# remmel/OcclusionFusion

Measured on AMD Instinct MI355X. Metric: fusion frames/sec (warp+integrate+solve), 640x480 depth -> 512^3 TSDF, higher is better.
Workload: dtype f32/f64

## Files before the change

occlusionfusion_amd/csrc/gn.hip:

```cpp
#include <math.h>
#include <stdlib.h>
#include <string.h>
#include <algorithm>
#include <chrono>
#include <array>
#include <condition_variable>
#include <memory>
#include <mutex>
#include <thread>
#include <type_traits>
#include <utility>
#include <cstdlib>
#include <cstdio>
#include <vector>

#include "ofx_common.h"

namespace ofx {

constexpr int kBlk = 256;
#ifndef OFX_KPROJ
#define OFX_KPROJ 4
#endif
constexpr int kProj = OFX_KPROJ;
// ... 1699 lines not shown
        const double z = M[a][b] / (dr[a] * dc[b]);
        const double err = (double)(float)h16(z) - z;
        e2 += 2.0 * err * err;
      }
    }
  s_e[t] = e2;
  __syncthreads();
  if (t < 64) {
    double sum = 0.0;
    for (int i = t; i < T; i += 64) sum += s_e[i];
    sum = wave_sum(sum);
    if (t == 0) s_sig = sqrt(sum) + 0x1p-10;
  }
  __syncthreads();
  OFX_AS_STAMP(3)
  const double sig = s_sig;
  auto b16 = [](_Float16 h) { return __builtin_bit_cast(uint16_t, h); };
#pragma unroll
  for (int a = 0; a < NA; ++a)
#pragma unroll
    for (int b = 0; b < NB; ++b) {
      const int R = tr + TR * a, C = tc + TC * b;
      if (R >= n || C >= kAsD) continue;
      if (C >= n) {
        s_z[R * kAsD + C] = 0;
      } else if (R == C) {
        s_z[R * kAsD + C] = b16(bad ? (_Float16)(R < 6 * kCS ? 1.0f : 0.0f) : h16(1.0 + sig));
      } else if (R < C) {
        const uint16_t h = b16(bad ? (_Float16)0.0f : h16(M[a][b] / (dr[a] * dc[b])));
        s_z[R * kAsD + C] = h;
        s_z[C * kAsD + R] = h;
      }
    }
  if (tc == 0)
#pragma unroll
    for (int a = 0; a < NA; ++a) {
      const int R = tr + TR * a;
      if (R < kAsD) g.as_dsc[(int64_t)c * kAsD + R] = R < n ? (float)dr[a] : 0.f;
      if (R < kAsD && g.as_one) as_tab_at(g.as_tab, g.as_tab_cap).dsc[(int64_t)c * kAsD + R] = R < n ? (float)dr[a] : 0.f;
      if (R < n) g.as_rsc[s_dst[R]] = (float)dr[a];
    }
  __syncthreads();
  OFX_AS_STAMP(4)
  for (int i = t; i < n * kAsK; i += T) {
    const int R = i / kAsK, k = i % kAsK;
    const int d = s_dst[R], cp = d / kAsRS, rs = d % kAsRS;
    reinterpret_cast<uint4*>(g.as_slab)[((int64_t)cp * kAsK + k) * kAsRS + rs] =
        reinterpret_cast<const uint4*>(s_z + R * kAsD)[k];
  }
  if (g.as_one) {
    uint4* sl = as_tab_at(g.as_tab, g.as_tab_cap).slab + (int64_t)c * kAsK * kAsD;
    for (int i = t; i < n * kAsK; i += T) {
      const int k = i / n, R = i - k * n;
      sl[(int64_t)k * kAsD + R] = reinterpret_cast<const uint4*>(s_z + R * kAsD)[k];
    }
  }
  if (t < kCS) g.racc[c * kCS + t] = 0.0;
  OFX_AS_STAMP(5)
#undef OFX_AS_STAMP
}

typedef double as_d4 __attribute__((ext_vector_type(4)));
constexpr int kNT = (kAsD + 15) / 16, kNP = 16 * kNT, kInvT = 64 * kNT;
__device__ __forceinline__ void as_invert_mfma(const GnDev& g, const double* __restrict__ A, int c, int t) {
  constexpr int kPanel = 16 * kNP;
  constexpr int kGJ = (2 * kPanel + 2 * 16 * 17) * 8, kZ = kAsD * kAsD * 2;
  __shared__ __attribute__((aligned(16))) char s_buf[kGJ > kZ ? kGJ : kZ];
  __shared__ int s_dom[kAsDN];
  __shared__ int s_sl[kAsDN][kAsDN];
  __shared__ int s_dst[kAsD];
  __shared__ double s_d[kNP], s_e[kInvT];
  __shared__ double s_sig;
  double* s_C = reinterpret_cast<double*>(s_buf);
  double* s_P = s_C + 2 * kPanel;
  uint16_t* s_z = reinterpret_cast<uint16_t*>(s_buf);
  const int l = t & 63, lr = l >> 4, lc = l & 15;
  const int w = __builtin_amdgcn_readfirstlane(t >> 6);
#ifdef OFX_STAMPS
#define OFX_AS_STAMP(k) \
  if (t == 0 && g.stamps) g.stamps[((int64_t)63 * g.nwg_row + c) * 8 + (k)] = __builtin_amdgcn_s_memtime();
#else
#define OFX_AS_STAMP(k)
#endif
  OFX_AS_STAMP(0)
  if (t < kAsDN) s_dom[t] = g.as_dom[c * kAsDN + t];
  if (t < kAsD) s_dst[t] = g.as_dst[(int64_t)c * kAsD + t];
  __syncthreads();
  int nd = 0;
  for (int i = 0; i < kAsDN; ++i) nd += s_dom[i] >= 0 ? 1 : 0;
  for (int q = t; q < kAsDN * kAsDN; q += kInvT) {
    const int i = q / kAsDN, j = q % kAsDN;
    s_sl[i][j] = (i < nd && j < nd) ? g.map[(int64_t)s_dom[i] * g.N + s_dom[j]] - 1 : -1;
  }
  __syncthreads();
  const int n = 6 * nd;
  const int C0 = 16 * w + lc;
  auto slot = [&](int R, int C) { return (R < n && C < n) ? s_sl[min(R / 6, kAsDN - 1)][min(C / 6, kAsDN - 1)] : -1; };
  as_d4 acc[kNT];
#pragma unroll
  for (int i = 0; i < kNT; ++i)
#pragma unroll
    for (int r = 0; r < 4; ++r) {
      const int R = 16 * i + lr + 4 * r;
      const int sl = slot(R, C0);
      acc[i][r] = A[36 * (int64_t)(sl >= 0 ? sl : 0) + 6 * (R % 6) + C0 % 6];
      if (r == 3) __builtin_amdgcn_sched_barrier(0);
    }
// ... 105 lines not shown
  __syncthreads();
  auto h16 = [](double z) -> _Float16 { return (_Float16)(float)z; };
  auto b16 = [](_Float16 h) { return __builtin_bit_cast(uint16_t, h); };
  double e2 = 0.0;
  const double dC = s_d[C0];
#pragma unroll
  for (int i = 0; i < kNT; ++i)
#pragma unroll
    for (int r = 0; r < 4; ++r) {
      const int R = 16 * i + lr + 4 * r;
      if (R >= n || C0 >= kAsD) continue;
      if (C0 >= n) {
        s_z[R * kAsD + C0] = 0;
      } else if (R < C0) {
        const double z = bad ? 0.0 : acc[i][r] / (s_d[R] * dC);
        const _Float16 h = h16(z);
        const double err = (double)(float)h - z;
        e2 += 2.0 * err * err;
        s_z[R * kAsD + C0] = b16(h);
        s_z[C0 * kAsD + R] = b16(h);
      }
      if (r == 3) __builtin_amdgcn_sched_barrier(0);
    }
  s_e[t] = e2;
  __syncthreads();
  if (t < 64) {
    double sum = 0.0;
    for (int i = t; i < kInvT; i += 64) sum += s_e[i];
    sum = wave_sum(sum);
    if (t == 0) s_sig = sqrt(sum) + 0x1p-10;
  }
  __syncthreads();
  OFX_AS_STAMP(3)
  const double sig = s_sig;
  if (t < n) s_z[t * kAsD + t] = b16(bad ? (_Float16)(t < 6 * kCS ? 1.0f : 0.0f) : h16(1.0 + sig));
  if (t < kAsD) {
    const double dr = s_d[t];
    g.as_dsc[(int64_t)c * kAsD + t] = t < n ? (float)dr : 0.f;
    if (g.as_one) as_tab_at(g.as_tab, g.as_tab_cap).dsc[(int64_t)c * kAsD + t] = t < n ? (float)dr : 0.f;
    if (t < n) g.as_rsc[s_dst[t]] = (float)dr;
  }
  __syncthreads();
  OFX_AS_STAMP(4)
  for (int i = t; i < n * kAsK; i += kInvT) {
    const int R = i / kAsK, k = i % kAsK;
    const int d = s_dst[R], cp = d / kAsRS, rs = d % kAsRS;
    reinterpret_cast<uint4*>(g.as_slab)[((int64_t)cp * kAsK + k) * kAsRS + rs] =
        reinterpret_cast<const uint4*>(s_z + R * kAsD)[k];
  }
  if (g.as_one) {
    uint4* sl = as_tab_at(g.as_tab, g.as_tab_cap).slab + (int64_t)c * kAsK * kAsD;
    for (int i = t; i < n * kAsK; i += kInvT) {
      const int k = i / n, R = i - k * n;
      sl[(int64_t)k * kAsD + R] = reinterpret_cast<const uint4*>(s_z + R * kAsD)[k];
    }
  }
  if (t < kCS) g.racc[c * kCS + t] = 0.0;
  OFX_AS_STAMP(5)
#undef OFX_AS_STAMP
}

constexpr int kAsInvTC = 16;
template <bool kMfma>
__global__ __launch_bounds__(kMfma ? kInvT : 16 * kAsInvTC) void k_as_invert(GnDev g, const double* __restrict__ A,
                                                                                   const double* __restrict__ rhs) {
  const int c = blockIdx.x, t = threadIdx.x;
  if (g.flags[F_STOPPED]) return;
  if constexpr (kMfma) as_invert_mfma(g, A, c, t);
  else as_invert_body<16, kAsInvTC>(g, A, c, t);
  if (!g.warm_now && t < 6 * kCS) {
    const int64_t o = 6 * (int64_t)c * kCS + t;
    const double v[V_N] = {0.0, rhs[o], 0.0, 0.0, 0.0, 0.0, 0.0, 0.0};
    store_rec(g.st, o, v);
  }
  if (c == 0 && t == 0) { g.flags[F_DONE] = 0; g.flags[F_PCG_IT] = 0; g.flags[F_PCG_CNT] = 0; g.flags[F_REFRESH] = 0; }
}

template <bool kTest, int kL>
__global__ __launch_bounds__(kAsRS * kL) void k_as_apply(const int32_t* stopw, const int32_t* meta, const int32_t* gat,
                                                        const uint16_t* slab, const double* in, double* out,
                                                        const int32_t* src, const float* dsc, const float* rsc) {
  constexpr int kT = kAsRS * kL;
  constexpr int kG = (kAsGat + kT - 1) / kT;
  constexpr int kKL = (kAsK + kL - 1) / kL;
  __shared__ __attribute__((aligned(16))) double s_w[kAsSrc * kAsD];
  __shared__ double s_seg[kAsRS];
  const int c = blockIdx.x, t = threadIdx.x, lane = t & 63;
  const int sg = t / kL, hl = t % kL;
  const int32_t* mt = meta + (int64_t)c * kAsMeta;
  int stop = 0;
  if (kTest) stop = stopw[(int64_t)c * 64 + lane];
  const int nrs = mt[0];
  int gn[kG], sv[kG];
#pragma unroll
  for (int j = 0; j < kG; ++j) {
    const int i = min(kT * j + t, kAsGat - 1);
    gn[j] = gat[(int64_t)c * kAsGat + i];
    sv[j] = src[c * kAsSrc + min(i / kAsDN, kAsSrc - 1)];
  }
  const int sl = mt[64 + sg];
  const float rscale = rsc[(int64_t)c * kAsRS + sg];
  const int rr = t < 6 * kCS ? t : 6 * kCS - 1;
  const int o0 = mt[2 + rr], o1 = mt[3 + rr];
  asm volatile("" ::: "memory");
  if (kTest) {
    stop = __builtin_amdgcn_readfirstlane(stop);
    if (stop != 0) return;
// ... 836 lines not shown
  double thr_new = 0.0, th_cur = 1e300;
  auto shift = [](int s) {
    const int e = s < 40 ? s : 2 * s - 40;
    const int k = e & 3;
    const double c = k == 0 ? 1.0 : k == 1 ? 0.84089641525371454303 : k == 2 ? 0.70710678118654752440
                                                                            : 0.59460355750136053336;
    return ldexp(c, -(e >> 2));
  };
  if (wv == 0 && hw == 0 && etol > 0.0) {
    const double rca = 1.0 / alpha;
    const double diag = kFirst ? rca : rca + beta * ralpha_prev;
    const double e2 = kFirst ? 0.0 : beta * ralpha_prev * ralpha_prev;
    const double sig = shift(lane);
    double d = (diag - sig) - (kFirst ? 0.0 : e2 / sd.x);
    if (fabs(d) < 1e-300) d = -1e-300;
    const double c = (kFirst ? 0.0 : sd.y) + (d < 0.0 ? 1.0 : 0.0);
    sd_new = make_double2(d, c);
    const uint64_t free_ = __ballot(c == 0.0);
    const double th = free_ ? shift(__ffsll((unsigned long long)free_) - 1) : 0.0;
    th_cur = th;
    const double tu = fmin(th, th_prev);
    thr_new = (etol * etol) * tu;
  }
  auto lead_stores = [&]() {
    if (lead) {
      sc_w[kScAlpha + 2 + par_] = 1.0 / alpha; sc_w[kScGamma + 2 + par_] = 1.0 / gam; flags_w[F_PCG_CNT] = cnt + 1;
      sc_w[kScAlpha + 4 + par_] = thr_new;
      if (etol > 0.0) sc_w[kScScal + S_TH_CUR] = th_cur;
    }
    if (wv == 0 && hw == 0 && etol > 0.0) reinterpret_cast<double2*>(sc_w + kScSturm)[lane] = sd_new;
    if (kFirst && lead) sc_w[kScScal + S_BB] = bb;
  };
  OFX_STAMP(2)
  OFX_STAMPX(6)
  double nc;
  if (kWave) {
#pragma unroll
    for (int j = 0; j < kNB; ++j) {
      const bool ok = (j ? bl1 : bl0).x >= 0;
      const int slot = kW2 ? 64 * hw + lane : j * 64 + lane;
      double x[6];
#pragma unroll
      for (int k = 0; k < 3; ++k) { x[2 * k] = xb[j][k].x; x[2 * k + 1] = xb[j][k].y; }
#pragma unroll
      for (int i = 0; i < 6; ++i) {
        const double2 b01 = ab[j][3 * i], b23 = ab[j][3 * i + 1], b45 = ab[j][3 * i + 2];
        const double t = fma(b45.y, x[5], fma(b45.x, x[4], fma(b23.y, x[3], fma(b23.x, x[2], fma(b01.y, x[1], b01.x * x[0])))));
        s_prod[slot * 6 + i] = ok ? t : 0.0;
      }
    }
    OFX_STAMP(3)
    if (kW2) {
      __builtin_amdgcn_s_waitcnt(0xC07F);
      __builtin_amdgcn_s_barrier();
    } else {
      wave_lds_sync();
    }
    const int len = b1 - b0;
    const double* sp = s_prod + (b0 - wb0) * 6 + qc;
    double tv[kRowMax];
#pragma unroll
    for (int k = 0; k < kRowMax; ++k) tv[k] = sp[6 * k];
    __builtin_amdgcn_sched_barrier(0);
    double a = 0.0;
#pragma unroll
    for (int k = 0; k < kRowMax; ++k) a += k < len ? tv[k] : 0.0;
    nc = a;
  } else {
    double n[6];
    row_spmv(g, b0, b1, q, mc, n);
    nc = pick6(n, qc);
  }
  OFX_STAMP(4)
  double d[kPcgStreams] = {0.0, 0.0, 0.0, 0.0};
  {
    const double zz = fma(beta, v[V_Z], nc);
    const double qq = fma(beta, v[V_Q], m);
    const double sv = fma(beta, v[V_S], v[V_W]);
    const double p = fma(beta, v[V_P], v[V_U]);
    const double rn = fma(-alpha, sv, v[V_R]);
    const double un = fma(-alpha, qq, v[V_U]);
    const double w2 = fma(-alpha, zz, v[V_W]);
    if (own) {
      const double nv[V_N] = {fma(alpha, p, v[V_X]), rn, un, zz, qq, sv, p, w2};
      if (w0) store_rec(stw, o, nv);
      if (kAS) {
        if (w0) reinterpret_cast<__attribute__((address_space(1))) double*>(addr(mcl_v))[o] = w2;
      } else {
        s_v[hw][6 * r + q] = w2;
      }
      d[0] = rn * un; d[1] = w2 * un; d[2] = rn * rn; d[3] = p * p;
    }
  }
  OFX_STAMP(5)
  if (!kAS) wave_lds_sync();
  if constexpr (kAS) {
  } else if (kW2) {
    double hsum = 0.0;
    if (own) {
      double2 vv[kCD / 4];
      const double2* sv2 = reinterpret_cast<const double2*>(&s_v[hw][4 * (kCD / 8) * hw]);
#pragma unroll
      for (int i = 0; i < kCD / 4; ++i) vv[i] = sv2[i];
      __builtin_amdgcn_sched_barrier(0);
      double a[4] = {0.0, 0.0, 0.0, 0.0};
#pragma unroll
      for (int kk = 0; kk < kCD / 8; ++kk) {
        const float4 t = mreg[kk];
        a[0] = fma((double)t.x, vv[2 * kk].x, a[0]);
        a[1] = fma((double)t.y, vv[2 * kk].y, a[1]);
        a[2] = fma((double)t.z, vv[2 * kk + 1].x, a[2]);
        a[3] = fma((double)t.w, vv[2 * kk + 1].y, a[3]);
      }
      hsum = (a[0] + a[1]) + (a[2] + a[3]);
    }
    if (hw == 1) s_half[lane] = hsum;
    __builtin_amdgcn_s_waitcnt(0xC07F);
    __builtin_amdgcn_s_barrier();
    if (w0 && own) mn[o] = hsum + s_half[lane];
  } else if (own) {
    double a[4] = {0.0, 0.0, 0.0, 0.0};
#pragma unroll
    for (int k = 0; k < kCD / 4; ++k) {
      const float4 t = mreg[k];
      a[0] = fma((double)t.x, s_v[0][4 * k], a[0]);
      a[1] = fma((double)t.y, s_v[0][4 * k + 1], a[1]);
      a[2] = fma((double)t.z, s_v[0][4 * k + 2], a[2]);
      a[3] = fma((double)t.w, s_v[0][4 * k + 3], a[3]);
    }
    mn[o] = (a[0] + a[1]) + (a[2] + a[3]);
  }
  OFX_STAMP(6)
  if (!w0) {
    if (kW2) {
      const double s2 = wave_sum(d[2]), s3 = wave_sum(d[3]);
      if (lane == 0) { Pn[2 * ns + wv] = s2; Pn[3 * ns + wv] = s3; }
    }
    return;
  }
  d[0] = wave_sum(d[0]);
  d[1] = wave_sum(d[1]);
  if (!kW2) { d[2] = wave_sum(d[2]); d[3] = wave_sum(d[3]); }
  if (lane == 0) {
    Pn[wv] = d[0]; Pn[ns + wv] = d[1];
    if (!kW2) { Pn[2 * ns + wv] = d[2]; Pn[3 * ns + wv] = d[3]; }
  }
  lead_stores();
  OFX_STAMP(7)
}

__device__ __forceinline__ void as_lds_barrier() {
  __builtin_amdgcn_s_waitcnt(0xC07F);
  __builtin_amdgcn_s_barrier();
}
#ifdef OFX_STAMPS
#define OFX_AS_ITER_STAMP(k, cn) \
  if (lane == 0 && g.stamps && (cn) < 64) g.stamps[((int64_t)(cn) * nwg + c) * 8 + (k)] = __builtin_amdgcn_s_memtime();
#else
#define OFX_AS_ITER_STAMP(k, cn)
#endif
template <bool kFirst, int kU, bool kRowSplit>
__global__ __launch_bounds__(kAsIterT) void k_as_iter(const int32_t* stopw, const double* Pc, const double* st,
                                                      const double* sc, const char* tab, int cap, int xcd_per, int nwg,
                                                      int ep, const PcgIt* gp, int gn_iter) {
  const PcgIt& g = *gp;
  constexpr int kNs = 128 * kU;
  constexpr int kS2W = 5 * 64;
  __shared__ __attribute__((aligned(16))) double s_m[kGS * 6];
  __shared__ __attribute__((aligned(16))) double s_prod[(kGB + kRowMax) * 6];
  __shared__ __attribute__((aligned(16))) double s_w[kAsD];
  __shared__ int s_leave;
  __shared__ double s_ab[2];
  const int t = threadIdx.x, lane = t & 63;
  const int wave = __builtin_amdgcn_readfirstlane(t >> 6);
  const int c = xcd_per > 0 ? (int)(blockIdx.x & 7) * xcd_per + (int)(blockIdx.x >> 3) : (int)blockIdx.x;
  if (c >= nwg) return;
  const AsTabP tp = as_tab_at(const_cast<char*>(tab), cap);
  const int par_ = (int)((reinterpret_cast<uintptr_t>(sc) >> 3) & 1);
  const double* scb = sc - par_;
  const int32_t* rt = tp.row + (int64_t)c * kGRow;
  const double* yr = tp.y + (int64_t)par_ * cap * kAsD;
  if (wave >= 8) {
    const int tb = t - kGB;
    int stop_ep = stopw[(int64_t)c * 64 + lane];
    const int nb = rt[26];
    typedef double gd2 __attribute__((ext_vector_type(2)));
    const __attribute__((address_space(1))) gd2* A2 =
        reinterpret_cast<const __attribute__((address_space(1))) gd2*>(reinterpret_cast<const uint64_t*>(scb)[kScAop]);
    if (kRowSplit) {
      constexpr int kP = (kGB * 6 + kGB - 1) / kGB;
      int2 be[kP];
#pragma unroll
      for (int j = 0; j < kP; ++j) be[j] = tp.blk[(int64_t)c * kGB + (tb + kGB * j) / 6];
      asm volatile("" ::: "memory");
      stop_ep = __builtin_amdgcn_readfirstlane(stop_ep);
      if (stop_ep != 0) return;
      double2 ar[kP][3];
#pragma unroll
      for (int j = 0; j < kP; ++j)
        if (tb - lane + kGB * j < 6 * nb)
#pragma unroll
          for (int k = 0; k < 3; ++k) {
            const gd2 x = A2[18 * (int64_t)be[j].x + 3 * ((tb + kGB * j) % 6) + k];
            ar[j][k] = make_double2(x.x, x.y);
          }
      as_lds_barrier();
#pragma unroll
      for (int j = 0; j < kP; ++j) {
        const int pp = tb + kGB * j;
        if (pp < 6 * nb) {
          const int k = be[j].y >> 5;
          double x[6];
#pragma unroll
          for (int q = 0; q < 6; ++q) x[q] = s_m[6 * k + q];
          const double2 b01 = ar[j][0], b23 = ar[j][1], b45 = ar[j][2];
          s_prod[pp] = fma(b45.y, x[5], fma(b45.x, x[4], fma(b23.y, x[3], fma(b23.x, x[2], fma(b01.y, x[1], b01.x * x[0])))));
        }
      }
      as_lds_barrier();
      as_lds_barrier();
      return;
    }
    const int2 be = tp.blk[(int64_t)c * kGB + tb];
    asm volatile("" ::: "memory");
    stop_ep = __builtin_amdgcn_readfirstlane(stop_ep);
    if (stop_ep != 0) return;
    const __attribute__((address_space(1))) gd2* b = A2 + 18 * (int64_t)be.x;
    const bool any = tb - lane < nb;
    double2 ab[18];
    if (any)
#pragma unroll
      for (int k = 0; k < 18; ++k) { const gd2 x = b[k]; ab[k] = make_double2(x.x, x.y); }
    as_lds_barrier();
    if (any && tb < nb) {
      const int k = be.y >> 5;
      double x[6];
#pragma unroll
      for (int j = 0; j < 6; ++j) x[j] = s_m[6 * k + j];
#pragma unroll
      for (int i = 0; i < 6; ++i) {
        const double2 b01 = ab[3 * i], b23 = ab[3 * i + 1], b45 = ab[3 * i + 2];
        s_prod[tb * 6 + i] =
            fma(b45.y, x[5], fma(b45.x, x[4], fma(b23.y, x[3], fma(b23.x, x[2], fma(b01.y, x[1], b01.x * x[0])))));
      }
    }
    as_lds_barrier();
    as_lds_barrier();
    return;
  }
  if (wave >= 3) {
    const int ts = t - 192;
    int stop_ep = stopw[(int64_t)c * 64 + lane];
    const int k2 = ts < kGS ? ts : kGS - 1;
    const int4 cn = tp.con[(int64_t)c * kGS + k2];
    const int nd = rt[25], ns = rt[27];
    const int ry = min(ts >> 1, kAsD - 1), hl = ts & 1;
    asm volatile("" ::: "memory");
    stop_ep = __builtin_amdgcn_readfirstlane(stop_ep);
    if (stop_ep != 0) return;
    auto gather = [&](int4 e4, double mv[6]) {
      double2 cz[4][3];
      {
        const int e[4] = {e4.x, e4.y, e4.z, e4.w};
#pragma unroll
        for (int j = 0; j < 4; ++j) {
#ifndef OFX_AS_NOSKIP
          if (j == 0 || e[j] >= 0) {
#pragma unroll
            for (int k = 0; k < 3; ++k) cz[j][k] = reinterpret_cast<const double2*>(yr + e[j])[k];
          } else {
#pragma unroll
            for (int k = 0; k < 3; ++k) cz[j][k] = make_double2(0.0, 0.0);
          }
#else
          const double2* p = reinterpret_cast<const double2*>(yr + (e[j] >= 0 ? e[j] : e[0]));
#pragma unroll
          for (int k = 0; k < 3; ++k) cz[j][k] = p[k];
#endif
        }
      }
      asm volatile("" ::: "memory");
#pragma unroll
      for (int k = 0; k < 3; ++k) {
        const int e[4] = {e4.x, e4.y, e4.z, e4.w};
        double mx = 0.0, my = 0.0;
#pragma unroll
        for (int j = 0; j < 4; ++j) { mx += e[j] >= 0 ? cz[j][k].x : 0.0; my += e[j] >= 0 ? cz[j][k].y : 0.0; }
        mv[2 * k] = mx; mv[2 * k + 1] = my;
      }
    };
    if (ts - lane < ns) {
      double mv[6];
      gather(cn, mv);
      if (ts < ns)
#pragma unroll
        for (int j = 0; j < 6; ++j) s_m[6 * ts + j] = mv[j];
    }
    if (ns > kS2W)
      for (int kk = ts + kS2W; kk < ns; kk += kS2W) {
        double mv[6];
        gather(tp.con[(int64_t)c * kGS + kk], mv);
#pragma unroll
        for (int j = 0; j < 6; ++j) s_m[6 * kk + j] = mv[j];
      }
    as_lds_barrier();
    uint4 z[9];
#pragma unroll
    for (int k = 0; k < 9; ++k) z[k] = tp.slab[((int64_t)c * kAsK + 9 * hl + k) * kAsD + ry];
    const float dsc_r = tp.dsc[(int64_t)c * kAsD + ry];
    as_lds_barrier();
    as_lds_barrier();
    if (s_leave) return;
    const double2* w2p = reinterpret_cast<const double2*>(s_w);
    double a0 = 0.0, a1 = 0.0, a2 = 0.0, a3 = 0.0;
    auto lo = [](uint32_t u) { return (double)(float)__builtin_bit_cast(_Float16, (uint16_t)(u & 0xFFFFu)); };
    auto hi = [](uint32_t u) { return (double)(float)__builtin_bit_cast(_Float16, (uint16_t)(u >> 16)); };
#pragma unroll
    for (int k = 0; k < 9; ++k) {
      const int kw = 9 * hl + k;
      const double2 p0 = w2p[4 * kw], p1 = w2p[4 * kw + 1], p2 = w2p[4 * kw + 2], p3 = w2p[4 * kw + 3];
      a0 = fma(lo(z[k].x), p0.x, a0);
      a1 = fma(hi(z[k].x), p0.y, a1);
      a2 = fma(lo(z[k].y), p1.x, a2);
      a3 = fma(hi(z[k].y), p1.y, a3);
      a0 = fma(lo(z[k].z), p2.x, a0);
      a1 = fma(hi(z[k].z), p2.y, a1);
      a2 = fma(lo(z[k].w), p3.x, a2);
      a3 = fma(hi(z[k].w), p3.y, a3);
    }
    double dot = (a0 + a1) + (a2 + a3);
    dot += dpp_mov<0xB1>(dot);
    if (hl == 0 && ts < 2 * kAsD && (ts >> 1) < 6 * nd)
      tp.y[(int64_t)(par_ ^ 1) * cap * kAsD + (int64_t)c * kAsD + (ts >> 1)] = (double)dsc_r * dot;
    return;
  }
  const int jr = wave, r = lane >> 3, q = lane & 7;
#ifdef OFX_STAMPS
  const uint64_t t_entry = __builtin_amdgcn_s_memtime();
#endif
  const bool own = q < 6;
  const int qc = own ? q : 5;
  const int l = 8 * jr + r;
  const int row = c * kCS + r;
  const int64_t o = 6 * (int64_t)row + qc;
  int stop_ep = stopw[(int64_t)c * 64 + lane];
  double2 tpp[kPcgStreams][kU];
  double own_p[kPcgStreams];
  int cnt = 0;
  double2 ra = make_double2(0.0, 0.0), rtb = ra, rg = ra, sd = ra, tols = ra;
  double bb_stored = 0.0, th_prev = 0.0;
  if (jr == 0) {
#pragma unroll
    for (int k = 0; k < kPcgStreams; ++k)
#pragma unroll
      for (int u = 0; u < kU; ++u) tpp[k][u] = *reinterpret_cast<const double2*>(Pc + k * kNs + 2 * (lane + 64 * u));
#pragma unroll
    for (int k = 0; k < kPcgStreams; ++k) own_p[k] = Pc[k * kNs + c];
    cnt = reinterpret_cast<const int32_t*>(scb + kScFlags)[F_PCG_CNT];
    ra = *reinterpret_cast<const double2*>(scb + kScAlpha + 2);
    rtb = *reinterpret_cast<const double2*>(scb + kScAlpha + 4);
    rg = *reinterpret_cast<const double2*>(scb + kScGamma + 2);
    sd = reinterpret_cast<const double2*>(scb + kScSturm)[lane];
    bb_stored = scb[kScScal + S_BB];
    th_prev = scb[kScScal + S_TH_PREV];
    tols = *reinterpret_cast<const double2*>(scb + kScTol);
  }
  const int nd = rt[25];
  const int rs = rt[l], re = rt[l + 1], rk = rt[32 + l];
  const float dsc_l = tp.dsc[(int64_t)c * kAsD + 6 * l + qc];
  double v[V_N];
  double wg = 0.0, zg = 0.0;
  const int gi = (c * kAsRing + (l >= kCS ? l - kCS : 0)) * 6 + qc;
  if (jr == 0) {
    load_rec(st, o, v);
  } else if (kFirst) {
    const double* w0v = reinterpret_cast<const double*>(reinterpret_cast<const uint64_t*>(scb)[kScMcl]);
    wg = w0v[6 * (int64_t)rt[64 + l] + qc];
    zg = 0.0;
  } else {
    const double2 gz = tp.gh[gi];
    wg = gz.x;
    zg = gz.y;
  }
  asm volatile("" ::: "memory");
  stop_ep = __builtin_amdgcn_readfirstlane(stop_ep);
  if (stop_ep != 0) return;
// ... 126 lines not shown
  };
  if (c == 0 && etol > 0.0) {
    const double rca = 1.0 / alpha;
    const double diag = kFirst ? rca : rca + beta * ralpha_prev;
    const double e2 = kFirst ? 0.0 : beta * ralpha_prev * ralpha_prev;
    const double sig = shift(lane);
    double dd = (diag - sig) - (kFirst ? 0.0 : e2 / sd.x);
    if (fabs(dd) < 1e-300) dd = -1e-300;
    const double cc = (kFirst ? 0.0 : sd.y) + (dd < 0.0 ? 1.0 : 0.0);
    sd_new = make_double2(dd, cc);
    const uint64_t free_ = __ballot(cc == 0.0);
    const double th = free_ ? shift(__ffsll((unsigned long long)free_) - 1) : 0.0;
    th_cur = th;
    const double tu = fmin(th, th_prev);
    thr_new = (etol * etol) * tu;
  }
  double* Pn = const_cast<double*>(Pc) + (par_ ? -kPcgStreams : kPcgStreams) * (int64_t)kNs;
#pragma unroll
  for (int k = 0; k < kPcgStreams; ++k) d[k] = wave_sum(d[k]);
  if (lane == 0) { Pn[c] = d[0]; Pn[kNs + c] = d[1]; Pn[2 * kNs + c] = d[2]; Pn[3 * kNs + c] = d[3]; }
  double* sc_w = const_cast<double*>(scb);
  int32_t* flags_w = reinterpret_cast<int32_t*>(sc_w + kScFlags);
  if (lead) {
    sc_w[kScAlpha + 2 + par_] = 1.0 / alpha; sc_w[kScGamma + 2 + par_] = 1.0 / gam; flags_w[F_PCG_CNT] = cnt + 1;
    sc_w[kScAlpha + 4 + par_] = thr_new;
    if (etol > 0.0) sc_w[kScScal + S_TH_CUR] = th_cur;
  }
  if (c == 0 && etol > 0.0) reinterpret_cast<double2*>(sc_w + kScSturm)[lane] = sd_new;
  if (kFirst && lead) sc_w[kScScal + S_BB] = bb;
  OFX_AS_ITER_STAMP(6, cnt)
}

template <bool kGather>
__global__ __launch_bounds__(kAsIterT) void k_as_w0(GnDev g, const double* rhs, int xcd_per) {
  __shared__ __attribute__((aligned(16))) double s_m[kGS * 6];
  __shared__ __attribute__((aligned(16))) double s_prod[(kGB + kRowMax) * 6];
  __shared__ __attribute__((aligned(16))) double s_w[kAsD];
  asm volatile("" :: "s"(g.as_tab), "s"(g.as_tab_cap), "s"(g.N), "s"(g.flags), "s"(g.m1), "s"(g.Aop), "s"(g.st),
               "s"(g.stopw), "s"(g.ep), "s"(g.pcs), "s"(rhs), "s"(g.part_p), "s"(g.part_b), "s"(g.nw_pad), "s"(g.as_w));
  const int t = threadIdx.x, lane = t & 63;
  const int wave = __builtin_amdgcn_readfirstlane(t >> 6);
  const int nwg = g.N / kCS;
  const int c = xcd_per > 0 ? (int)(blockIdx.x & 7) * xcd_per + (int)(blockIdx.x >> 3) : (int)blockIdx.x;
  if (c >= nwg) return;
  const AsTabP tp = as_tab_at(g.as_tab, g.as_tab_cap);
  const int32_t* rt = tp.row + (int64_t)c * kGRow;
  const int stopped = g.flags[F_STOPPED];
  if (wave >= 8) {
    const int tb = t - kGB;
    constexpr int kP = (kGB * 6 + kGB - 1) / kGB;
    int2 be[kP];
#pragma unroll
    for (int j = 0; j < kP; ++j) be[j] = tp.blk[(int64_t)c * kGB + (tb + kGB * j) / 6];
    const int nb = rt[26];
    asm volatile("" ::: "memory");
    if (stopped) return;
    const double2* A2 = reinterpret_cast<const double2*>(g.Aop);
    double2 ar[kP][3];
#pragma unroll
    for (int j = 0; j < kP; ++j)
      if (tb - lane + kGB * j < 6 * nb)
#pragma unroll
        for (int k = 0; k < 3; ++k) ar[j][k] = A2[18 * (int64_t)be[j].x + 3 * ((tb + kGB * j) % 6) + k];
    as_lds_barrier();
#pragma unroll
    for (int j = 0; j < kP; ++j) {
      const int pp = tb + kGB * j;
      if (pp < 6 * nb) {
        const int k = be[j].y >> 5;
        double x[6];
#pragma unroll
        for (int q = 0; q < 6; ++q) x[q] = s_m[6 * k + q];
        const double2 b01 = ar[j][0], b23 = ar[j][1], b45 = ar[j][2];
        s_prod[pp] = ((b01.x * x[0] + b01.y * x[1]) + (b23.x * x[2] + b23.y * x[3])) + (b45.x * x[4] + b45.y * x[5]);
      }
    }
    as_lds_barrier();
    as_lds_barrier();
    return;
  }
  if (wave >= 3) {
    constexpr int kS2W = 5 * 64;
    const int ts = t - 192;
    const int k2 = ts < kGS ? ts : kGS - 1;
    int s2u = 0;
    int4 cn = make_int4(-1, -1, -1, -1);
    if (kGather) cn = tp.con[(int64_t)c * kGS + k2];
    else s2u = tp.s2n[(int64_t)c * kGS + k2];
    const int nd = rt[25], ns = rt[27];
    const int ry = min(ts >> 1, kAsD - 1), hl = ts & 1;
    asm volatile("" ::: "memory");
    if (stopped) return;
    const double* yr = tp.y + (int64_t)g.as_tab_cap * kAsD;
    auto gather = [&](int4 e4, int u, double mv[6]) {
      if (kGather) {
        const int e[4] = {e4.x, e4.y, e4.z, e4.w};
        double2 cz[4][3];
#pragma unroll
        for (int j = 0; j < 4; ++j) {
          if (j == 0 || e[j] >= 0) {
#pragma unroll
            for (int k = 0; k < 3; ++k) cz[j][k] = reinterpret_cast<const double2*>(yr + e[j])[k];
          } else {
#pragma unroll
            for (int k = 0; k < 3; ++k) cz[j][k] = make_double2(0.0, 0.0);
          }
        }
        asm volatile("" ::: "memory");
#pragma unroll
        for (int k = 0; k < 3; ++k) {
          double mx = 0.0, my = 0.0;
#pragma unroll
          for (int j = 0; j < 4; ++j) { mx += e[j] >= 0 ? cz[j][k].x : 0.0; my += e[j] >= 0 ? cz[j][k].y : 0.0; }
          mv[2 * k] = mx; mv[2 * k + 1] = my;
        }
      } else {
        const double2* p = reinterpret_cast<const double2*>(g.m1 + 6 * (int64_t)u);
#pragma unroll
        for (int k = 0; k < 3; ++k) { const double2 x = p[k]; mv[2 * k] = x.x; mv[2 * k + 1] = x.y; }
      }
    };
    if (ts - lane < ns) {
      double mv[6];
      gather(cn, s2u, mv);
      if (ts < ns)
#pragma unroll
        for (int k = 0; k < 6; ++k) s_m[6 * ts + k] = mv[k];
    }
    if (ns > kS2W)
      for (int kk = ts + kS2W; kk < ns; kk += kS2W) {
        double mv[6];
        gather(kGather ? tp.con[(int64_t)c * kGS + kk] : make_int4(-1, -1, -1, -1),
               kGather ? 0 : tp.s2n[(int64_t)c * kGS + kk], mv);
#pragma unroll
        for (int k = 0; k < 6; ++k) s_m[6 * kk + k] = mv[k];
      }
    as_lds_barrier();
    uint4 z[9];
#pragma unroll
    for (int k = 0; k < 9; ++k) z[k] = tp.slab[((int64_t)c * kAsK + 9 * hl + k) * kAsD + ry];
    const float dsc_r = tp.dsc[(int64_t)c * kAsD + ry];
    as_lds_barrier();
    as_lds_barrier();
    const double2* w2p = reinterpret_cast<const double2*>(s_w);
    double a0 = 0.0, a1 = 0.0, a2 = 0.0, a3 = 0.0;
    auto lo = [](uint32_t u) { return (double)(float)__builtin_bit_cast(_Float16, (uint16_t)(u & 0xFFFFu)); };
    auto hi = [](uint32_t u) { return (double)(float)__builtin_bit_cast(_Float16, (uint16_t)(u >> 16)); };
#pragma unroll
    for (int k = 0; k < 9; ++k) {
      const int kw = 9 * hl + k;
      const double2 p0 = w2p[4 * kw], p1 = w2p[4 * kw + 1], p2 = w2p[4 * kw + 2], p3 = w2p[4 * kw + 3];
      a0 = fma(lo(z[k].x), p0.x, a0);
      a1 = fma(hi(z[k].x), p0.y, a1);
      a2 = fma(lo(z[k].y), p1.x, a2);
      a3 = fma(hi(z[k].y), p1.y, a3);
      a0 = fma(lo(z[k].z), p2.x, a0);
      a1 = fma(hi(z[k].z), p2.y, a1);
      a2 = fma(lo(z[k].w), p3.x, a2);
      a3 = fma(hi(z[k].w), p3.y, a3);
    }
    double dot = (a0 + a1) + (a2 + a3);
    dot += dpp_mov<0xB1>(dot);
    if (hl == 0 && ts < 2 * kAsD && (ts >> 1) < 6 * nd)
      tp.y[(int64_t)c * kAsD + (ts >> 1)] = (double)dsc_r * dot;
    return;
  }
  const int jr = wave, r = lane >> 3, q = lane & 7;
  const bool own = q < 6;
  const int qc = own ? q : 5;
  const int l = 8 * jr + r;
  const int row = c * kCS + r;
  const int64_t o = 6 * (int64_t)row + q, oc = 6 * (int64_t)row + qc;
  const int nd = rt[25];
  const int rs = rt[l], re = rt[l + 1];
  const float dsc_l = tp.dsc[(int64_t)c * kAsD + 6 * l + qc];
  const int rk = rt[32 + l];
  double v[V_N];
  double u_as = 0.0, bo = 0.0, th_cur_old = 0.0;
  if (jr == 0) {
    load_rec(g.st, oc, v);
    if (!kGather) u_as = g.m1[oc];
    bo = rhs[oc];
    th_cur_old = g.pcs[kScScal + S_TH_CUR];
  }
  asm volatile("" ::: "memory");
  if (stopped) {
    if (jr == 0) {
      g.stopw[(int64_t)c * 64 + lane] = g.ep;
      if (c == 0 && lane == 0) w0_lead_stores(g, th_cur_old, true, true);
    }
    return;
  }
  as_lds_barrier();
  if (kGather && jr == 0) u_as = s_m[6 * rk + qc];
  as_lds_barrier();
  const int len = l < nd ? re - rs : 0;
  const double* sp = s_prod + rs * 6 + qc;
  double tv[kRowMax];
#pragma unroll
  for (int k = 0; k < kRowMax; ++k) tv[k] = sp[6 * k];
  double w = 0.0;
#pragma unroll
  for (int k = 0; k < kRowMax; ++k) w += k < len ? tv[k] : 0.0;
  double d[4] = {0.0, 0.0, 0.0, 0.0};
  if (jr == 0 && own) {
    v[V_U] = u_as;
    v[V_W] = w;
    store_rec(g.st, o, v);
    g.as_w[o] = w;
    d[0] = v[V_R] * v[V_U]; d[1] = w * v[V_U]; d[2] = v[V_R] * v[V_R]; d[3] = bo * bo;
  }
  if (own) s_w[6 * l + q] = l < nd ? w * (double)dsc_l : 0.0;
  as_lds_barrier();
  if (jr != 0) return;
#pragma unroll
  for (int k = 0; k < 4; ++k) d[k] = wave_sum(d[k]);
  const int ns = g.nw_pad;
  if (lane == 0) {
    g.part_p[c] = d[0]; g.part_p[ns + c] = d[1]; g.part_p[2 * ns + c] = d[2];
    g.part_p[3 * ns + c] = 0.0;
    g.part_b[c] = d[3];
  }
  if (c == 0)
    for (int i = nwg + lane; i < ns; i += 64) {
#pragma unroll
      for (int k = 0; k < 2 * kPcgStreams; ++k) g.part_p[k * ns + i] = 0.0;
      g.part_b[i] = 0.0;
    }
  g.stopw[(int64_t)c * 64 + lane] = 0;
  if (c == 0 && lane == 0) w0_lead_stores(g, th_cur_old, true, true);
}

template <int KU>
__global__ __launch_bounds__(512) void k_as_proj2(GnDev g, const double* rhs, int xcd_per) {
  __shared__ __attribute__((aligned(16))) double s_w[kAsD];
  __shared__ double s_c[kProj];
  __shared__ int s_fin;
  asm volatile("" :: "s"(g.as_tab), "s"(g.as_tab_cap), "s"(g.N), "s"(g.flags), "s"(g.n_prev), "s"(g.xh), "s"(g.th),
               "s"(g.part_p), "s"(g.nw_pad), "s"(g.stopw), "s"(g.ep), "s"(g.st), "s"(rhs));
  const int t = threadIdx.x, lane = t & 63;
  const int wave = __builtin_amdgcn_readfirstlane(t >> 6);
  const int nwg = g.N / kCS;
  const int c = xcd_per > 0 ? (int)(blockIdx.x & 7) * xcd_per + (int)(blockIdx.x >> 3) : (int)blockIdx.x;
  if (c >= nwg) return;
  const AsTabP tp = as_tab_at(g.as_tab, g.as_tab_cap);
  const int32_t* rt = tp.row + (int64_t)c * kGRow;
  const int stopped = g.flags[F_STOPPED];
  if (wave >= 3) {
    const int ts = t - 192;
    const int ry = min(ts >> 1, kAsD - 1), hl = ts & 1;
    const int nd = rt[25];
    uint4 z[9];
#pragma unroll
    for (int k = 0; k < 9; ++k) z[k] = tp.slab[((int64_t)c * kAsK + 9 * hl + k) * kAsD + ry];
    const float dsc_r = tp.dsc[(int64_t)c * kAsD + ry];
    asm volatile("" ::: "memory");
    if (stopped) return;
    as_lds_barrier();
    as_lds_barrier();
    const double2* w2p = reinterpret_cast<const double2*>(s_w);
    double a0 = 0.0, a1 = 0.0, a2 = 0.0, a3 = 0.0;
    auto lo = [](uint32_t u) { return (double)(float)__builtin_bit_cast(_Float16, (uint16_t)(u & 0xFFFFu)); };
    auto hi = [](uint32_t u) { return (double)(float)__builtin_bit_cast(_Float16, (uint16_t)(u >> 16)); };
#pragma unroll
    for (int k = 0; k < 9; ++k) {
      const int kw = 9 * hl + k;
      const double2 p0 = w2p[4 * kw], p1 = w2p[4 * kw + 1], p2 = w2p[4 * kw + 2], p3 = w2p[4 * kw + 3];
      a0 = fma(lo(z[k].x), p0.x, a0);
      a1 = fma(hi(z[k].x), p0.y, a1);
      a2 = fma(lo(z[k].y), p1.x, a2);
      a3 = fma(hi(z[k].y), p1.y, a3);
      a0 = fma(lo(z[k].z), p2.x, a0);
      a1 = fma(hi(z[k].z), p2.y, a1);
      a2 = fma(lo(z[k].w), p3.x, a2);
      a3 = fma(hi(z[k].w), p3.y, a3);
    }
    double dot = (a0 + a1) + (a2 + a3);
    dot += dpp_mov<0xB1>(dot);
    if (hl == 0 && ts < 2 * kAsD && (ts >> 1) < 6 * nd)
      tp.y[(int64_t)g.as_tab_cap * kAsD + (int64_t)c * kAsD + (ts >> 1)] = (double)dsc_r * dot;
    return;
  }
  const int jr = wave, r = lane >> 3, q = lane & 7;
  const bool own = q < 6;
  const int qc = own ? q : 5;
  const int l = 8 * jr + r;
  const int row = c * kCS + r;
  const int64_t o = 6 * (int64_t)row + q;
  const int nd = rt[25];
  const int64_t og = jr == 0 ? 6 * (int64_t)row + qc : 6 * (int64_t)rt[64 + l] + qc;
  const float dsc_l = tp.dsc[(int64_t)c * kAsD + 6 * l + qc];
  const int np = g.n_prev;
  const int64_t stride = 6 * (int64_t)g.N;
  const double rb = rhs[og];
  double xo[kProj], to[kProj];
#pragma unroll
  for (int j = 0; j < kProj; ++j) { xo[j] = jr == 0 ? g.xh[j * stride + og] : 0.0; to[j] = g.th[j * stride + og]; }
  double2 pt[kProjP][KU];
  if (jr == 0) load_streams2_padded<kProjP, KU>(g.part_p, g.nw_pad, pt);
  asm volatile("" ::: "memory");
  if (stopped) {
    if (jr == 0) g.stopw[(int64_t)c * 64 + lane] = g.ep;
    return;
  }
  if (jr == 0) {
    double cj[kProj];
    const bool fin = galerkin_coeffs<KU>(g, np, pt, cj);
    if (lane == 0) {
#pragma unroll
      for (int j = 0; j < kProj; ++j) s_c[j] = cj[j];
      s_fin = fin ? 1 : 0;
    }
  }
  as_lds_barrier();
  const bool fin = s_fin != 0;
  double xv = 0.0, rv = rb;
#pragma unroll
  for (int j = 0; j < kProj; ++j)
    if (j < np && fin) { const double cj = s_c[j]; xv += cj * xo[j]; rv -= cj * to[j]; }
  if (jr == 0 && own) {
    const double v[V_N] = {xv, rv, 0.0, 0.0, 0.0, 0.0, 0.0, 0.0};
    store_rec(g.st, o, v);
  }
  if (own) s_w[6 * l + q] = l < nd ? rv * (double)dsc_l : 0.0;
  as_lds_barrier();
}
// ... 1405 lines not shown
```

Before: 357.0.

## Spread the slab dot product over four lanes per row with swizzled slab layout

The per-row dot of the fp16 slab against the LDS weight vector moves from two lanes per row with uint4 loads to four lanes per row with uint2 loads. Each lane now holds 9 words and the partials are combined with two DPP reductions. The slab words are stored swizzled (y and z swapped) so each lane's uint2 pair lines up with its weights, and idle waves of the gather group take part of the dot. The intent is to lower the per-lane register load and latency of this tail, at the cost of more lanes, an extra DPP step, and a layout change every consumer of the slab must follow.

New measurement: 371.1 (median of 6 runs). 3.9% higher.

```diff
diff --git a/occlusionfusion_amd/csrc/gn.hip b/occlusionfusion_amd/csrc/gn.hip
--- a/occlusionfusion_amd/csrc/gn.hip
+++ b/occlusionfusion_amd/csrc/gn.hip
@@ -1775,7 +1775,8 @@
     uint4* sl = as_tab_at(g.as_tab, g.as_tab_cap).slab + (int64_t)c * kAsK * kAsD;
     for (int i = t; i < n * kAsK; i += T) {
       const int k = i / n, R = i - k * n;
-      sl[(int64_t)k * kAsD + R] = reinterpret_cast<const uint4*>(s_z + R * kAsD)[k];
+      const uint4 v = reinterpret_cast<const uint4*>(s_z + R * kAsD)[k];
+      sl[(int64_t)k * kAsD + R] = make_uint4(v.x, v.z, v.y, v.w);
     }
   }
   if (t < kCS) g.racc[c * kCS + t] = 0.0;
@@ -1987,7 +1988,8 @@
     uint4* sl = as_tab_at(g.as_tab, g.as_tab_cap).slab + (int64_t)c * kAsK * kAsD;
     for (int i = t; i < n * kAsK; i += kInvT) {
       const int k = i / n, R = i - k * n;
-      sl[(int64_t)k * kAsD + R] = reinterpret_cast<const uint4*>(s_z + R * kAsD)[k];
+      const uint4 v = reinterpret_cast<const uint4*>(s_z + R * kAsD)[k];
+      sl[(int64_t)k * kAsD + R] = make_uint4(v.x, v.z, v.y, v.w);
     }
   }
   if (t < kCS) g.racc[c * kCS + t] = 0.0;
@@ -2930,7 +2932,9 @@
     OFX_STAMP(3)
     if (kW2) {
       __builtin_amdgcn_s_waitcnt(0xC07F);
+      asm volatile("" ::: "memory");
       __builtin_amdgcn_s_barrier();
+      asm volatile("" ::: "memory");
     } else {
       wave_lds_sync();
     }
@@ -3029,7 +3033,64 @@
 
 __device__ __forceinline__ void as_lds_barrier() {
   __builtin_amdgcn_s_waitcnt(0xC07F);
+  asm volatile("" ::: "memory");
   __builtin_amdgcn_s_barrier();
+  asm volatile("" ::: "memory");
+}
+constexpr int kAsDotT = 4 * kAsD;
+constexpr int kDotBW = (kAsDotT - 5 * 64 + 63) / 64;
+static_assert(kDotBW >= 0 && kDotBW <= 8, "the dot's lanes fit waves 3-15");
+struct AsDotRow {
+  uint2 z[9];
+  float dsc;
+  int yd;
+};
+static_assert(kAsK == 18, "the dot's lanes take 9 words of their half each");
+__device__ __forceinline__ void as_dot_load(const AsTabP& tp, int c, int tq, AsDotRow& d) {
+  const int ry = min(tq >> 2, kAsD - 1), hl = (tq >> 1) & 1, g = tq & 1;
+  const uint2* sl = reinterpret_cast<const uint2*>(tp.slab + ((int64_t)c * kAsK + 9 * hl) * kAsD + ry) + g;
+#pragma unroll
+  for (int k = 0; k < 9; ++k) d.z[k] = sl[(int64_t)k * 2 * kAsD];
+  d.dsc = tp.dsc[(int64_t)c * kAsD + ry];
+  d.yd = c * kAsD + ry;
+}
+__device__ __forceinline__ void as_dot_cvt(const AsDotRow& d, double (&f)[36]) {
+#pragma unroll
+  for (int k = 0; k < 9; ++k) {
+    f[4 * k] = (double)(float)__builtin_bit_cast(_Float16, (uint16_t)(d.z[k].x & 0xFFFFu));
+    f[4 * k + 1] = (double)(float)__builtin_bit_cast(_Float16, (uint16_t)(d.z[k].x >> 16));
+    f[4 * k + 2] = (double)(float)__builtin_bit_cast(_Float16, (uint16_t)(d.z[k].y & 0xFFFFu));
+    f[4 * k + 3] = (double)(float)__builtin_bit_cast(_Float16, (uint16_t)(d.z[k].y >> 16));
+  }
+}
+__device__ __forceinline__ double as_dot_sum(const double (&f)[36], const double* s_w, int tq) {
+  const int hl = (tq >> 1) & 1, g = tq & 1;
+  const double2* w2p = reinterpret_cast<const double2*>(s_w) + 36 * hl + g;
+  double a = 0.0, b = 0.0;
+#pragma unroll
+  for (int k = 0; k < 9; ++k) {
+    const double2 p0 = w2p[4 * k], p2 = w2p[4 * k + 2];
+    a = fma(f[4 * k], p0.x, a);
+    b = fma(f[4 * k + 1], p0.y, b);
+    a = fma(f[4 * k + 2], p2.x, a);
+    b = fma(f[4 * k + 3], p2.y, b);
+  }
+  double dot = a + b;
+  dot += dpp_mov<0xB1>(dot);
+  dot += dpp_mov<0x4E>(dot);
+  return dot;
+}
+__device__ __forceinline__ void as_dot_tail(const AsDotRow& d, const double* s_w, const int* leave, int tq, int nd,
+                                            double* y_w) {
+  as_lds_barrier();
+  double f[36];
+  as_dot_cvt(d, f);
+#pragma unroll
+  for (int k = 0; k < 36; ++k) asm volatile("" : "+v"(f[k]));
+  as_lds_barrier();
+  if (leave && *leave) return;
+  const double dot = as_dot_sum(f, s_w, tq);
+  if ((tq & 3) == 0 && tq < kAsDotT && (tq >> 2) < 6 * nd) y_w[d.yd] = (double)d.dsc * dot;
 }
 #ifdef OFX_STAMPS
 #define OFX_AS_ITER_STAMP(k, cn) \
@@ -3061,7 +3122,7 @@
   if (wave >= 8) {
     const int tb = t - kGB;
     int stop_ep = stopw[(int64_t)c * 64 + lane];
-    const int nb = rt[26];
+    const int nb = rt[26], nd = rt[25];
     typedef double gd2 __attribute__((ext_vector_type(2)));
     const __attribute__((address_space(1))) gd2* A2 =
         reinterpret_cast<const __attribute__((address_space(1))) gd2*>(reinterpret_cast<const uint64_t*>(scb)[kScAop]);
@@ -3073,6 +3134,7 @@
       asm volatile("" ::: "memory");
       stop_ep = __builtin_amdgcn_readfirstlane(stop_ep);
       if (stop_ep != 0) return;
+      __builtin_amdgcn_s_waitcnt(0x0F70);
       double2 ar[kP][3];
 #pragma unroll
       for (int j = 0; j < kP; ++j)
@@ -3094,6 +3156,12 @@
           const double2 b01 = ar[j][0], b23 = ar[j][1], b45 = ar[j][2];
           s_prod[pp] = fma(b45.y, x[5], fma(b45.x, x[4], fma(b23.y, x[3], fma(b23.x, x[2], fma(b01.y, x[1], b01.x * x[0])))));
         }
+      }
+      if (wave < 8 + kDotBW) {
+        AsDotRow dr;
+        as_dot_load(tp, c, t - 192, dr);
+        as_dot_tail(dr, s_w, &s_leave, t - 192, nd, tp.y + (int64_t)(par_ ^ 1) * cap * kAsD);
+        return;
       }
       as_lds_barrier();
       as_lds_barrier();
@@ -3122,6 +3190,12 @@
             fma(b45.y, x[5], fma(b45.x, x[4], fma(b23.y, x[3], fma(b23.x, x[2], fma(b01.y, x[1], b01.x * x[0])))));
       }
     }
+    if (wave < 8 + kDotBW) {
+      AsDotRow dr;
+      as_dot_load(tp, c, t - 192, dr);
+      as_dot_tail(dr, s_w, &s_leave, t - 192, nd, tp.y + (int64_t)(par_ ^ 1) * cap * kAsD);
+      return;
+    }
     as_lds_barrier();
     as_lds_barrier();
     return;
@@ -3132,7 +3206,6 @@
     const int k2 = ts < kGS ? ts : kGS - 1;
     const int4 cn = tp.con[(int64_t)c * kGS + k2];
     const int nd = rt[25], ns = rt[27];
-    const int ry = min(ts >> 1, kAsD - 1), hl = ts & 1;
     asm volatile("" ::: "memory");
     stop_ep = __builtin_amdgcn_readfirstlane(stop_ep);
     if (stop_ep != 0) return;
@@ -3182,34 +3255,9 @@
         for (int j = 0; j < 6; ++j) s_m[6 * kk + j] = mv[j];
       }
     as_lds_barrier();
-    uint4 z[9];
-#pragma unroll
-    for (int k = 0; k < 9; ++k) z[k] = tp.slab[((int64_t)c * kAsK + 9 * hl + k) * kAsD + ry];
-    const float dsc_r = tp.dsc[(int64_t)c * kAsD + ry];
-    as_lds_barrier();
-    as_lds_barrier();
-    if (s_leave) return;
-    const double2* w2p = reinterpret_cast<const double2*>(s_w);
-    double a0 = 0.0, a1 = 0.0, a2 = 0.0, a3 = 0.0;
-    auto lo = [](uint32_t u) { return (double)(float)__builtin_bit_cast(_Float16, (uint16_t)(u & 0xFFFFu)); };
-    auto hi = [](uint32_t u) { return (double)(float)__builtin_bit_cast(_Float16, (uint16_t)(u >> 16)); };
-#pragma unroll
-    for (int k = 0; k < 9; ++k) {
-      const int kw = 9 * hl + k;
-      const double2 p0 = w2p[4 * kw], p1 = w2p[4 * kw + 1], p2 = w2p[4 * kw + 2], p3 = w2p[4 * kw + 3];
-      a0 = fma(lo(z[k].x), p0.x, a0);
-      a1 = fma(hi(z[k].x), p0.y, a1);
-      a2 = fma(lo(z[k].y), p1.x, a2);
-      a3 = fma(hi(z[k].y), p1.y, a3);
-      a0 = fma(lo(z[k].z), p2.x, a0);
-      a1 = fma(hi(z[k].z), p2.y, a1);
-      a2 = fma(lo(z[k].w), p3.x, a2);
-      a3 = fma(hi(z[k].w), p3.y, a3);
-    }
-    double dot = (a0 + a1) + (a2 + a3);
-    dot += dpp_mov<0xB1>(dot);
-    if (hl == 0 && ts < 2 * kAsD && (ts >> 1) < 6 * nd)
-      tp.y[(int64_t)(par_ ^ 1) * cap * kAsD + (int64_t)c * kAsD + (ts >> 1)] = (double)dsc_r * dot;
+    AsDotRow dr;
+    as_dot_load(tp, c, ts, dr);
+    as_dot_tail(dr, s_w, &s_leave, ts, nd, tp.y + (int64_t)(par_ ^ 1) * cap * kAsD);
     return;
   }
   const int jr = wave, r = lane >> 3, q = lane & 7;
@@ -3442,9 +3490,10 @@
     int2 be[kP];
 #pragma unroll
     for (int j = 0; j < kP; ++j) be[j] = tp.blk[(int64_t)c * kGB + (tb + kGB * j) / 6];
-    const int nb = rt[26];
+    const int nb = rt[26], nd = rt[25];
     asm volatile("" ::: "memory");
     if (stopped) return;
+    __builtin_amdgcn_s_waitcnt(0x0F70);
     const double2* A2 = reinterpret_cast<const double2*>(g.Aop);
     double2 ar[kP][3];
 #pragma unroll
@@ -3464,6 +3513,12 @@
         const double2 b01 = ar[j][0], b23 = ar[j][1], b45 = ar[j][2];
         s_prod[pp] = ((b01.x * x[0] + b01.y * x[1]) + (b23.x * x[2] + b23.y * x[3])) + (b45.x * x[4] + b45.y * x[5]);
       }
+    }
+    if (wave < 8 + kDotBW) {
+      AsDotRow dr;
+      as_dot_load(tp, c, t - 192, dr);
+      as_dot_tail(dr, s_w, nullptr, t - 192, nd, tp.y);
+      return;
     }
     as_lds_barrier();
     as_lds_barrier();
@@ -3478,7 +3533,6 @@
     if (kGather) cn = tp.con[(int64_t)c * kGS + k2];
     else s2u = tp.s2n[(int64_t)c * kGS + k2];
     const int nd = rt[25], ns = rt[27];
-    const int ry = min(ts >> 1, kAsD - 1), hl = ts & 1;
     asm volatile("" ::: "memory");
     if (stopped) return;
     const double* yr = tp.y + (int64_t)g.as_tab_cap * kAsD;
@@ -3526,33 +3580,9 @@
         for (int k = 0; k < 6; ++k) s_m[6 * kk + k] = mv[k];
       }
     as_lds_barrier();
-    uint4 z[9];
-#pragma unroll
-    for (int k = 0; k < 9; ++k) z[k] = tp.slab[((int64_t)c * kAsK + 9 * hl + k) * kAsD + ry];
-    const float dsc_r = tp.dsc[(int64_t)c * kAsD + ry];
-    as_lds_barrier();
-    as_lds_barrier();
-    const double2* w2p = reinterpret_cast<const double2*>(s_w);
-    double a0 = 0.0, a1 = 0.0, a2 = 0.0, a3 = 0.0;
-    auto lo = [](uint32_t u) { return (double)(float)__builtin_bit_cast(_Float16, (uint16_t)(u & 0xFFFFu)); };
-    auto hi = [](uint32_t u) { return (double)(float)__builtin_bit_cast(_Float16, (uint16_t)(u >> 16)); };
-#pragma unroll
-    for (int k = 0; k < 9; ++k) {
-      const int kw = 9 * hl + k;
-      const double2 p0 = w2p[4 * kw], p1 = w2p[4 * kw + 1], p2 = w2p[4 * kw + 2], p3 = w2p[4 * kw + 3];
-      a0 = fma(lo(z[k].x), p0.x, a0);
-      a1 = fma(hi(z[k].x), p0.y, a1);
-      a2 = fma(lo(z[k].y), p1.x, a2);
-      a3 = fma(hi(z[k].y), p1.y, a3);
-      a0 = fma(lo(z[k].z), p2.x, a0);
-      a1 = fma(hi(z[k].z), p2.y, a1);
-      a2 = fma(lo(z[k].w), p3.x, a2);
-      a3 = fma(hi(z[k].w), p3.y, a3);
-    }
-    double dot = (a0 + a1) + (a2 + a3);
-    dot += dpp_mov<0xB1>(dot);
-    if (hl == 0 && ts < 2 * kAsD && (ts >> 1) < 6 * nd)
-      tp.y[(int64_t)c * kAsD + (ts >> 1)] = (double)dsc_r * dot;
+    AsDotRow dr;
+    as_dot_load(tp, c, ts, dr);
+    as_dot_tail(dr, s_w, nullptr, ts, nd, tp.y);
     return;
   }
   const int jr = wave, r = lane >> 3, q = lane & 7;
@@ -3658,10 +3688,10 @@
       const double2 p0 = w2p[4 * kw], p1 = w2p[4 * kw + 1], p2 = w2p[4 * kw + 2], p3 = w2p[4 * kw + 3];
       a0 = fma(lo(z[k].x), p0.x, a0);
       a1 = fma(hi(z[k].x), p0.y, a1);
-      a2 = fma(lo(z[k].y), p1.x, a2);
-      a3 = fma(hi(z[k].y), p1.y, a3);
-      a0 = fma(lo(z[k].z), p2.x, a0);
-      a1 = fma(hi(z[k].z), p2.y, a1);
+      a2 = fma(lo(z[k].z), p1.x, a2);
+      a3 = fma(hi(z[k].z), p1.y, a3);
+      a0 = fma(lo(z[k].y), p2.x, a0);
+      a1 = fma(hi(z[k].y), p2.y, a1);
       a2 = fma(lo(z[k].w), p3.x, a2);
       a3 = fma(hi(z[k].w), p3.y, a3);
     }
```
